# 18281818221/kalle-audio

Measured on AMD Instinct MI355X. Metric: audio-seconds/sec (node) DiT train step, 10s@12.5Hz x1024 latents, higher is better.
Workload: dtype bf16; 1 GPU; DiT train step (fwd+bwd+allreduce+Adam), 24 blocks D=1536 h=24, 10 s @ 12.5 Hz x 1024 latents (T=125+1 prepend), S=130 x 768 cross-attn cond; DiT shape chosen by this build (reference defines none); global_batch=256, per_gpu_batch=256, parallelism=dp1, objective=v, io_channels=1024, global_cond_type=prepend

## Files before the change

### kalle_audio_amd/csrc/gemm2.hip

```cpp
#include <stdio.h>
#include <stdlib.h>
#include <string.h>

#include <algorithm>
#include <functional>
#include <type_traits>
#include <utility>

#include "gemm_common.h"
#include "../../include/kalle_hip.h"

namespace {

constexpr int BK2 = 64;
#define GPTR(p) ((const __attribute__((address_space(1))) void*)(p))

__device__ __attribute__((aligned(64))) const unsigned kalle_zero_block[16] = {0, 0, 0, 0, 0, 0, 0, 0, 0, 0, 0, 0, 0, 0, 0, 0};

template <bool KM, int R, int NW>
struct Loader {
    static constexpr int PER_WAVE = (R / 8) / NW;
    const bf16_t* src[PER_WAVE];
    int64_t kstep;

// ... 56 lines not shown
        if (t == tail_t) issue_tail(region, wave, lane, kvalid);
        else issue(region, wave);
    }
};

template <int OFF>
__device__ __forceinline__ i32x4 lds_b128(unsigned a) {
    i32x4 r;
    asm volatile("ds_read_b128 %0, %1 offset:%2" : "=v"(r) : "v"(a), "n"(OFF));
    return r;
}
__device__ __forceinline__ i32x2 lds_tr(unsigned a) {
    i32x2 r;
    asm volatile("ds_read_b64_tr_b16 %0, %1" : "=v"(r) : "v"(a));
    return r;
}

template <bool KM, int R>
struct Reader {
    unsigned b0[2], b1[2];
    __device__ __forceinline__ void init(int region_off, int rbase, int lane) {
#pragma unroll
        for (int s = 0; s < 2; ++s) {
            if constexpr (!KM) {
                const int row = rbase + (lane & 15);
                const int c = 4 * s + (lane >> 4);
                b0[s] = region_off + row * 128 + ((c ^ ((row >> 1) & 7)) << 4);
                b1[s] = 0;
            } else {
                constexpr int RB = 2 * R;
                const int g = lane >> 4, i = lane & 15;
                const int q = i >> 2, pp = i & 3;
                const int b = 4 * s + g;
                const int odd = b & 1;
                const int pos1 = 8 * b + (odd ? 4 : 0) + q;
                const int pos2 = 8 * b + (odd ? 0 : 4) + q;
                const int cl = (rbase >> 3) + (pp >> 1);
                const int hb = (pp & 1) * 8;
                b0[s] = region_off + pos1 * RB + ((cl ^ (2 * (pos1 & 7))) << 4) + hb;
                b1[s] = region_off + pos2 * RB + ((cl ^ (2 * (pos2 & 7))) << 4) + hb;
            }
        }
    }
    template <int S, int NTILE, int T0 = 0>
    __device__ __forceinline__ void read(unsigned so, i32x4 (&f)[NTILE]) const {
        if constexpr (!KM) {
            const unsigned a = b0[S] + so;
            f[0] = lds_b128<2048 * (T0 + 0)>(a);
            f[1] = lds_b128<2048 * (T0 + 1)>(a);
            f[2] = lds_b128<2048 * (T0 + 2)>(a);
            f[3] = lds_b128<2048 * (T0 + 3)>(a);
            if constexpr (NTILE == 8) {
                f[4] = lds_b128<2048 * (T0 + 4)>(a);
                f[5] = lds_b128<2048 * (T0 + 5)>(a);
                f[6] = lds_b128<2048 * (T0 + 6)>(a);
                f[7] = lds_b128<2048 * (T0 + 7)>(a);
            }
        } else {
            const unsigned a0 = b0[S] + so, a1 = b1[S] + so;
#pragma unroll
            for (int t = 0; t < NTILE; ++t) {
                const i32x2 lo = lds_tr(a0 ^ ((T0 + t) << 5));
                const i32x2 hi = lds_tr(a1 ^ ((T0 + t) << 5));
                f[t] = i32x4{lo[0], lo[1], hi[0], hi[1]};
            }
        }
    }
};

__device__ __forceinline__ void gemm_stamp(const GemmParams& p, int wave, int lane, int idx, int slot = -1) {
    if (p.stamps && (wave == 0 || wave == 7) && lane == 0)
        p.stamps[((int64_t)(slot < 0 ? (int)blockIdx.x : slot) * 2 + (wave ? 1 : 0)) * 8 + idx] = __builtin_amdgcn_s_memrealtime();
}

constexpr int EPI_DEPTH = 1;

struct NoHook { __device__ __forceinline__ void operator()() const {} };

__device__ __forceinline__ int pidx(int r, int c) { return r * 64 + (c ^ ((r & 1) << 2)); }

template <bool C_F32, int TM, int GLU = 0, typename Hook = NoHook>
__device__ __forceinline__ void wave_epilogue(const GemmParams& p, f32x4 (&acc)[TM][4], char* patch_base, int wave, int lane,
                                              int row0, int col0, Hook after_barrier = Hook{}, int stamp_slot = -1) {
    constexpr int DEPTH = EPI_DEPTH < TM ? EPI_DEPTH : TM;
    float* patch = reinterpret_cast<float*>(patch_base) + wave * (16 * 64);
    const int g = lane >> 4, li = lane & 15;
    const bool pre_res = C_F32 && GLU == 0 && !p.atomic && p.residual != nullptr;
    f32x4 rbuf[DEPTH][4];
    auto load_res = [&](int mt, f32x4 (&rv)[4]) {
#pragma unroll
        for (int i = 0; i < 4; ++i) {
            const int gm = row0 + 16 * mt + g + 4 * i, gn = col0 + 4 * li;
            rv[i] = f32x4{0.f, 0.f, 0.f, 0.f};
            if (gm < p.M && gn < p.N) rv[i] = *reinterpret_cast<const f32x4*>(p.residual + gemm_crow(p, gm) * p.ldr + gn);
        }
    };
    i32x4 hbuf[DEPTH][2][2];
    auto load_h = [&](int mt, i32x4 (&hv)[2][2]) {
        const int c8 = (lane & 7) * 8, j0 = col0 + c8;
#pragma unroll
        for (int half = 0; half < 2; ++half) {
            const int gm = row0 + 16 * mt + (lane >> 3) + 8 * half;
            hv[half][0] = i32x4{0, 0, 0, 0};
            hv[half][1] = i32x4{0, 0, 0, 0};
            if (gm < p.M && j0 < p.glu_inner) {
                const bf16_t* hp = static_cast<const bf16_t*>(p.glu_aux) + (int64_t)gm * 2 * p.glu_inner;
                hv[half][0] = *reinterpret_cast<const i32x4*>(hp + j0);
                hv[half][1] = *reinterpret_cast<const i32x4*>(hp + p.glu_inner + j0);
            }
        }
    };
    asm volatile("s_waitcnt lgkmcnt(0)" ::: "memory");
    __builtin_amdgcn_s_barrier();
    after_barrier();
    gemm_stamp(p, wave, lane, 3, stamp_slot);
#pragma unroll
    for (int d = 0; d < DEPTH; ++d) {
        if constexpr (GLU == 2) load_h(d, hbuf[d]);
        if (pre_res) load_res(d, rbuf[d]);
    }
    float sx[8], sg[8];
#pragma unroll
    for (int e = 0; e < 8; ++e) { sx[e] = 0.f; sg[e] = 0.f; }
    f32x4 bias4 = f32x4{0.f, 0.f, 0.f, 0.f}, bias8[2] = {f32x4{0.f, 0.f, 0.f, 0.f}, f32x4{0.f, 0.f, 0.f, 0.f}};
    float bx[8], bg[8];
#pragma unroll
    for (int e = 0; e < 8; ++e) { bx[e] = 0.f; bg[e] = 0.f; }
    if (p.bias) {
        if constexpr (GLU == 1) {
            const int j0 = col0 + (lane & 3) * 8;
            if (j0 < p.glu_inner) {
#pragma unroll
                for (int e = 0; e < 8; ++e) { bx[e] = p.bias[j0 + e]; bg[e] = p.bias[p.glu_inner + j0 + e]; }
            }
        } else if constexpr (GLU == 0) {
            if constexpr (C_F32) {
                if (!p.atomic && col0 + 4 * li < p.N) bias4 = *reinterpret_cast<const f32x4*>(p.bias + col0 + 4 * li);
            } else {
                const int gn = col0 + 8 * (lane & 7);
                if (gn < p.N) {
                    bias8[0] = *reinterpret_cast<const f32x4*>(p.bias + gn);
                    bias8[1] = *reinterpret_cast<const f32x4*>(p.bias + gn + 4);
                }
            }
        }
    }
#pragma unroll
    for (int mt = 0; mt < TM; ++mt) {
        const int slot = mt % DEPTH;
        f32x4 rcur[4];
        i32x4 hcur[2][2];
        if constexpr (GLU == 2) {
#pragma unroll
            for (int half = 0; half < 2; ++half) { hcur[half][0] = hbuf[slot][half][0]; hcur[half][1] = hbuf[slot][half][1]; }
            if (mt + DEPTH < TM) load_h(mt + DEPTH, hbuf[slot]);
        }
        if (pre_res) {
#pragma unroll
            for (int i = 0; i < 4; ++i) rcur[i] = rbuf[slot][i];
            if (mt + DEPTH < TM) load_res(mt + DEPTH, rbuf[slot]);
        }
#pragma unroll
        for (int nt = 0; nt < 4; ++nt)
#pragma unroll
            for (int r = 0; r < 4; ++r) patch[pidx(4 * g + r, 16 * nt + li)] = acc[mt][nt][r];
        asm volatile("s_waitcnt lgkmcnt(0)" ::: "memory");
        const int rbase = row0 + 16 * mt;
        if constexpr (GLU == 1) {
            const int r = lane >> 2, c8 = (lane & 3) * 8;
            const int gm = rbase + r, j0 = col0 + c8;
            if (gm < p.M && j0 < p.glu_inner) {
                float xv[8], gv[8];
#pragma unroll
                for (int e = 0; e < 8; ++e) { xv[e] = patch[pidx(r, c8 + e)]; gv[e] = patch[pidx(r, 32 + c8 + e)]; }
#pragma unroll
                for (int e = 0; e < 8; ++e) { xv[e] += bx[e]; gv[e] += bg[e]; }
                i32x4 hx, hg, av;
#pragma unroll
                for (int e = 0; e < 4; ++e) {
                    hx[e] = (int)pack_bf16x2(xv[2 * e], xv[2 * e + 1]);
                    hg[e] = (int)pack_bf16x2(gv[2 * e], gv[2 * e + 1]);
                    const float x0 = bf16lo((uint32_t)hx[e]), x1 = bf16hi((uint32_t)hx[e]);
                    const float g0 = bf16lo((uint32_t)hg[e]), g1 = bf16hi((uint32_t)hg[e]);
                    av[e] = (int)pack_bf16x2(x0 * siluf_(g0), x1 * siluf_(g1));
                }
                bf16_t* hp = reinterpret_cast<bf16_t*>(p.C) + (int64_t)gm * p.ldc;
                *reinterpret_cast<i32x4*>(hp + j0) = hx;
                *reinterpret_cast<i32x4*>(hp + p.glu_inner + j0) = hg;
                *reinterpret_cast<i32x4*>(static_cast<bf16_t*>(p.glu_aux) + (int64_t)gm * p.glu_inner + j0) = av;
            }
        } else if constexpr (GLU == 2) {
            const int c8 = (lane & 7) * 8, j0 = col0 + c8;
#pragma unroll
            for (int half = 0; half < 2; ++half) {
                const int r = (lane >> 3) + 8 * half;
                const int gm = rbase + r;
                if (gm < p.M && j0 < p.glu_inner) {
                    const i32x4 xv = hcur[half][0], gv = hcur[half][1];
                    i32x4 ox, og;
#pragma unroll
                    for (int e = 0; e < 4; ++e) {
                        const float x[2] = {bf16lo((uint32_t)xv[e]), bf16hi((uint32_t)xv[e])};
                        const float gg[2] = {bf16lo((uint32_t)gv[e]), bf16hi((uint32_t)gv[e])};
                        const float d[2] = {bf16_to_f32(f32_to_bf16(patch[pidx(r, c8 + 2 * e)] * p.alpha)),
                                            bf16_to_f32(f32_to_bf16(patch[pidx(r, c8 + 2 * e + 1)] * p.alpha))};
                        float dx[2], dg[2];
#pragma unroll
                        for (int q = 0; q < 2; ++q) {
                            const float sgm = sigmoidf_(gg[q]);
                            dx[q] = d[q] * gg[q] * sgm;
                            dg[q] = d[q] * x[q] * sgm * (1.f + gg[q] * (1.f - sgm));
                        }
                        ox[e] = (int)pack_bf16x2(dx[0], dx[1]);
                        og[e] = (int)pack_bf16x2(dg[0], dg[1]);
                        sx[2 * e] += bf16lo((uint32_t)ox[e]); sx[2 * e + 1] += bf16hi((uint32_t)ox[e]);
                        sg[2 * e] += bf16lo((uint32_t)og[e]); sg[2 * e + 1] += bf16hi((uint32_t)og[e]);
                    }
                    bf16_t* dp = reinterpret_cast<bf16_t*>(p.C) + (int64_t)gm * p.ldc;
                    *reinterpret_cast<i32x4*>(dp + j0) = ox;
                    *reinterpret_cast<i32x4*>(dp + p.glu_inner + j0) = og;
                }
            }
        } else if (p.atomic) {
            const int gn = col0 + lane;
#pragma unroll 4
            for (int r = 0; r < 16; ++r) {
                const int gm = rbase + r;
                if (gm < p.M && gn < p.N)
                    atomicAdd(reinterpret_cast<float*>(p.C) + (int64_t)gm * p.ldc + gn, patch[pidx(r, lane)] * p.alpha);
            }
        } else if constexpr (C_F32) {
#pragma unroll
            for (int i = 0; i < 4; ++i) {
                const int r = g + 4 * i;
                const int gm = rbase + r, gn = col0 + 4 * li;
                if (gm >= p.M || gn >= p.N) continue;
                const f32x4 pv = *reinterpret_cast<const f32x4*>(patch + pidx(r, 4 * li));
                float v[4] = {pv[0], pv[1], pv[2], pv[3]};
                const int64_t crow = gemm_crow(p, gm);
                gemm_epilogue4(p, gm, gn, crow, v, false, &bias4);
                if (pre_res) {
#pragma unroll
                    for (int j = 0; j < 4; ++j) v[j] += rcur[i][j];
                }
                float* cp = reinterpret_cast<float*>(p.C) + crow * p.ldc + gn;
                if (p.accumulate) {
                    const f32x4 c0 = *reinterpret_cast<const f32x4*>(cp);
#pragma unroll
                    for (int j = 0; j < 4; ++j) v[j] += c0[j];
                }
                *reinterpret_cast<f32x4*>(cp) = f32x4{v[0], v[1], v[2], v[3]};
            }
        } else {
#pragma unroll
            for (int half = 0; half < 2; ++half) {
                const int r = (lane >> 3) + 8 * half;
                const int gm = rbase + r, gn = col0 + 8 * (lane & 7);
                if (gm >= p.M || gn >= p.N) continue;
                const f32x4 p0 = *reinterpret_cast<const f32x4*>(patch + pidx(r, 8 * (lane & 7)));
                const f32x4 p1 = *reinterpret_cast<const f32x4*>(patch + pidx(r, 8 * (lane & 7) + 4));
                float v0[4] = {p0[0], p0[1], p0[2], p0[3]}, v1[4] = {p1[0], p1[1], p1[2], p1[3]};
                const int64_t crow = gemm_crow(p, gm);
                gemm_epilogue4(p, gm, gn, crow, v0, true, &bias8[0]);
                gemm_epilogue4(p, gm, gn + 4, crow, v1, true, &bias8[1]);
                i32x4 o;
                o[0] = (int)pack_bf16x2(v0[0], v0[1]);
                o[1] = (int)pack_bf16x2(v0[2], v0[3]);
                o[2] = (int)pack_bf16x2(v1[0], v1[1]);
                o[3] = (int)pack_bf16x2(v1[2], v1[3]);
                *reinterpret_cast<i32x4*>(reinterpret_cast<bf16_t*>(p.C) + crow * p.ldc + gn) = o;
            }
        }
        asm volatile("s_waitcnt lgkmcnt(0)" ::: "memory");
    }
    if constexpr (GLU == 2) {
        if (p.glu_dbias) {
#pragma unroll
            for (int e = 0; e < 8; ++e) {
#pragma unroll
                for (int o = 8; o < 64; o <<= 1) { sx[e] += __shfl_xor(sx[e], o, 64); sg[e] += __shfl_xor(sg[e], o, 64); }
            }
            const int j0 = col0 + (lane & 7) * 8;
            if (lane < 8 && j0 < p.glu_inner) {
#pragma unroll
                for (int e = 0; e < 8; ++e) {
                    atomicAdd(p.glu_dbias + j0 + e, sx[e]);
                    atomicAdd(p.glu_dbias + p.glu_inner + j0 + e, sg[e]);
                }
            }
        }
    }
    if (p.stamps) {
        gemm_stamp(p, wave, lane, 4, stamp_slot);
        asm volatile("s_waitcnt vmcnt(0)" ::: "memory");
        gemm_stamp(p, wave, lane, 5, stamp_slot);
    }
}

#define MFMA16(FA, FB)                                                                                         \
    _Pragma("unroll") for (int mt = 0; mt < 4; ++mt) _Pragma("unroll") for (int nt = 0; nt < 4; ++nt)          \
        acc[mt][nt] = __builtin_amdgcn_mfma_f32_16x16x32_bf16(__builtin_bit_cast(bf16x8, FA[mt]),              \
                                                              __builtin_bit_cast(bf16x8, FB[nt]), acc[mt][nt], 0, 0, 0)

template <bool A_KM, bool B_KM, bool C_F32, int WM, int WN, int TM, int GLU = 0, int NS = 3>
__global__ __launch_bounds__(WM * WN * 64, 2) void gemm2_kernel(GemmParams p) {
    static_assert(TM == 4, "wave tile is 64 x 64");
    constexpr int TN = 4;
    constexpr int NW = WM * WN;
    constexpr int BM = WM * TM * 16, BN = WN * TN * 16;
    constexpr int A_BYTES = BM * 128, B_BYTES = BN * 128, STAGE = A_BYTES + B_BYTES;
    extern __shared__ __attribute__((aligned(16))) char smem[];
    const unsigned lds0 = (unsigned)(size_t)LDS_PTR(char, smem);

    const int tid = threadIdx.x, lane = tid & 63;
    const int wave = __builtin_amdgcn_readfirstlane(tid >> 6);
    const int wm = wave / WN, wn = wave % WN;

    int tm, tn;
    gemm_tile_coords(blockIdx.x, gridDim.x, p.tiles_m, p.tiles_n, p.group_m, tm, tn);
    const int m0 = tm * BM, n0 = tn * BN;

    const int nk_all = (p.K + BK2 - 1) / BK2;
    const int kt0 = blockIdx.y * p.ktiles_per_split;
    const int nk = min(p.ktiles_per_split, nk_all - kt0);
    const int kvalid = p.K % BK2;
    const int tail_t = kvalid ? nk_all - 1 - kt0 : -1;

    f32x4 acc[TM][TN];
#pragma unroll
    for (int i = 0; i < TM; ++i)
#pragma unroll
        for (int j = 0; j < TN; ++j) acc[i][j] = f32x4{0.f, 0.f, 0.f, 0.f};

    Loader<A_KM, BM, NW> la;
    Loader<B_KM, BN, NW> lb;
    la.init(p.A, p.lda, p.M, m0, kt0 * BK2, wave, lane);
    lb.init(p.B, p.ldb, p.N, n0, kt0 * BK2, wave, lane, GLU == 1 ? p.glu_inner : 0, tn);
    const int arow = wm * TM * 16, bcol = wn * TN * 16;
    Reader<A_KM, BM> ra;
    Reader<B_KM, BN> rb;
    ra.init(lds0, arow, lane);
    rb.init(lds0 + A_BYTES, bcol, lane);

    {
    constexpr int PT = Loader<A_KM, BM, NW>::PER_WAVE + Loader<B_KM, BN, NW>::PER_WAVE;
    static_assert((NS - 2) * PT <= 63, "vmcnt is a 6-bit counter");
    {
        const int pre = nk < NS ? nk : NS;
#pragma unroll
        for (int t = 0; t < NS; ++t) {
            if (t < pre) {
                la.issue_at(smem + t * STAGE, wave, lane, t, tail_t, kvalid);
                lb.issue_at(smem + t * STAGE + A_BYTES, wave, lane, t, tail_t, kvalid);
            }
        }
        constexpr int PRE_KEEP = (NS - 1) * PT <= 63 ? NS - 1 : NS - 2;
        const int keep = pre - 1 < PRE_KEEP ? pre - 1 : PRE_KEEP;
        auto wait_keep = [&](auto self, auto c) {
            constexpr int C = decltype(c)::value;
            if (keep == C) asm volatile("s_waitcnt vmcnt(%0)" ::"n"(C * PT) : "memory");
            if constexpr (C > 0) self(self, std::integral_constant<int, C - 1>{});
        };
        wait_keep(wait_keep, std::integral_constant<int, PRE_KEEP>{});
    }
    __builtin_amdgcn_s_barrier();
    __builtin_amdgcn_sched_barrier(0);

    i32x4 fa0[4], fb0[4], fa1[4], fb1[4];
    ra.template read<0, 4>(0, fa0);
    rb.template read<0, 4>(0, fb0);

    unsigned so_cur = 0, so_nxt = STAGE;
    int kt = 0;

    auto iteration = [&](auto issue_c, auto next_c, auto keep_c) {
        constexpr bool ISSUE = decltype(issue_c)::value, NEXT = decltype(next_c)::value;
        constexpr int KEEP = decltype(keep_c)::value;
        asm volatile("s_waitcnt lgkmcnt(0)" ::: "memory");
        __builtin_amdgcn_sched_barrier(0);
// ... 210 lines not shown
template <bool A_KM, bool B_KM, bool C_F32, int WM, int WN, int TM, int GLU = 0, int NS = 3>
int launch2(const GemmParams& p, hipStream_t st) {
    constexpr int BM = WM * TM * 16, BN = WN * 64;
    constexpr int lds = NS * (BM + BN) * 128;
    static_assert(lds <= 160 * 1024, "LDS per workgroup");
    static std::atomic<uint64_t> lds_ok{0};
    kalle_allow_lds(reinterpret_cast<const void*>(gemm2_kernel<A_KM, B_KM, C_F32, WM, WN, TM, GLU, NS>), lds, lds_ok);
    dim3 grid(p.tiles_m * p.tiles_n, p.splits), block(WM * WN * 64);
    KALLE_LAUNCH((gemm2_kernel<A_KM, B_KM, C_F32, WM, WN, TM, GLU, NS>), grid, block, lds, st, p);
    return kalle_check_launch();
}



constexpr int GEMM3_LDS = 2 * (256 + 256) * 128 + 8 * 16 * 64 * 4;

static int kalle_cu_count() {
    static std::atomic<int> cached[64];
    int dev = 0;
    (void)hipGetDevice(&dev);
    int v = cached[dev & 63].load(std::memory_order_relaxed);
    if (v > 0) return v;
    hipDeviceProp_t prop;
    v = hipGetDeviceProperties(&prop, dev) == hipSuccess && prop.multiProcessorCount > 0 ? prop.multiProcessorCount : 256;
    v &= ~7;
    if (v < 8) v = 8;
    cached[dev & 63].store(v, std::memory_order_relaxed);
    return v;
}

#define MFMA32(FA, FB)                                                                                         \
    _Pragma("unroll") for (int mt = 0; mt < 8; ++mt) _Pragma("unroll") for (int nt = 0; nt < 4; ++nt)          \
        acc[mt][nt] = __builtin_amdgcn_mfma_f32_16x16x32_bf16(__builtin_bit_cast(bf16x8, FA[mt]),              \
                                                              __builtin_bit_cast(bf16x8, FB[nt]), acc[mt][nt], 0, 0, 0)

constexpr int SCHED_SETS = 256;
constexpr int SCHED_LINE = 32;
__device__ int kalle_gemm_sched[SCHED_SETS][9 * SCHED_LINE];

__device__ __forceinline__ int sched_issue(int* sched, int xcd) { return atomicAdd(sched + xcd * SCHED_LINE, 1); }
__device__ __forceinline__ int sched_resolve(int xcd, int raw, int first_round, int ntiles) {
    const int id = xcd + 8 * (first_round + raw);
    return id < ntiles ? id : ntiles;
}
__device__ __forceinline__ void sched_leave(int* sched, int nwg) {
    if (atomicAdd(sched + 8 * SCHED_LINE, 1) == nwg - 1) {
#pragma unroll
        for (int i = 0; i < 9; ++i) atomicExch(sched + i * SCHED_LINE, 0);
    }
}

template <bool A_KM, bool B_KM, bool C_F32, int GLU, bool XCD_RASTER, bool PERSIST>
__device__ __forceinline__ void gemm3_tiles(const GemmParams& p, int tile0, int tstride, int tile_end, int ntiles_raster, int kt0,
                                            int nk) {
    const int kvalid = p.K % BK2;
    const int tail_t = kvalid ? (p.K + BK2 - 1) / BK2 - 1 - kt0 : -1;
    constexpr int WN = 4, TM = 8, NW = 8;
    constexpr int BM = 256, BN = 256;
    constexpr int A_BYTES = BM * 128, B_BYTES = BN * 128, STAGE = A_BYTES + B_BYTES;
    extern __shared__ __attribute__((aligned(16))) char smem[];
    const unsigned lds0 = (unsigned)(size_t)LDS_PTR(char, smem);

    const int tid = threadIdx.x, lane = tid & 63;
    const int wave = __builtin_amdgcn_readfirstlane(tid >> 6);
    const int wm = wave / WN, wn = wave % WN;
    const int arow = wm * 128, bcol = wn * 64;
    Loader<A_KM, BM, NW> la;
    Loader<B_KM, BN, NW> lb;
    Reader<A_KM, BM> ra;
    Reader<B_KM, BN> rb;
    ra.init(lds0, arow, lane);
    rb.init(lds0 + A_BYTES, bcol, lane);
    const bool late = wave >= NW / 2;
    if (late) __builtin_amdgcn_s_setprio(1);

    auto coords = [&](int tile, int& tm, int& tn) {
        if constexpr (XCD_RASTER) gemm_tile_coords(tile, ntiles_raster, p.tiles_m, p.tiles_n, p.group_m, tm, tn);
        else gemm_tile_coords_plain(tile, p.tiles_m, p.tiles_n, p.group_m, tm, tn);
    };
    auto init_loaders = [&](int tm, int tn, int kt_first) {
        la.init(p.A, p.lda, p.M, tm * BM, (kt0 + kt_first) * BK2, wave, lane);
        lb.init(p.B, p.ldb, p.N, tn * BN, (kt0 + kt_first) * BK2, wave, lane, GLU == 1 ? p.glu_inner : 0, tn);
    };
    bool prefetched = false;
    unsigned s0 = 0;

    int* const sched = PERSIST && p.sched_set > 0 ? &kalle_gemm_sched[p.sched_set - 1][0] : nullptr;
    int next_tile = tile_end;
    int drawn = 0;
    if constexpr (PERSIST) {
        if (sched && tid == 0) drawn = sched_issue(sched, blockIdx.x & 7);
    }
    volatile int* const mailbox = reinterpret_cast<volatile int*>(smem + 2 * STAGE);
    for (int tile = tile0; tile < tile_end; tile = next_tile) {
        int tm, tn;
        coords(tile, tm, tn);
        const int m0 = tm * BM, n0 = tn * BN;
        next_tile = PERSIST ? tile + tstride : tile_end;
        bool has_next = PERSIST && next_tile < tile_end;
        gemm_stamp(p, wave, lane, 0, tile);
        f32x4 acc[TM][4];
#pragma unroll
        for (int i = 0; i < TM; ++i)
#pragma unroll
            for (int j = 0; j < 4; ++j) acc[i][j] = f32x4{0.f, 0.f, 0.f, 0.f};

        if (!prefetched) {
            init_loaders(tm, tn, 0);
            la.issue_at(smem, wave, lane, 0, tail_t, kvalid);
            lb.issue_at(smem + A_BYTES, wave, lane, 0, tail_t, kvalid);
            s0 = 0;
            if (nk > 1) {
                la.issue_at(smem + STAGE, wave, lane, 1, tail_t, kvalid);
                lb.issue_at(smem + STAGE + A_BYTES, wave, lane, 1, tail_t, kvalid);
                asm volatile("s_waitcnt vmcnt(8)" ::: "memory");
            } else {
                asm volatile("s_waitcnt vmcnt(0)" ::: "memory");
            }
        } else if constexpr (PERSIST) {
            init_loaders(tm, tn, nk > 1 ? 2 : 1);
            asm volatile("s_waitcnt vmcnt(0)" ::: "memory");
        }
        if constexpr (PERSIST) {
            if (sched && tid == 0) {
                *mailbox = sched_resolve(blockIdx.x & 7, drawn, tstride >> 3, tile_end);
                asm volatile("s_waitcnt lgkmcnt(0)" ::: "memory");
            }
        }
        __builtin_amdgcn_s_barrier();
        __builtin_amdgcn_sched_barrier(0);
        if constexpr (PERSIST) {
            if (sched) {
                next_tile = __builtin_amdgcn_readfirstlane(*mailbox);
                has_next = next_tile < tile_end;
            }
        }
        gemm_stamp(p, wave, lane, 1, tile);

        i32x4 fa[8], fb[4];
        unsigned so_cur = s0;
        int kt = 0;
        ra.template read<0, 8>(so_cur, fa);
        rb.template read<0, 4>(so_cur, fb);

        auto iteration = [&](auto issue_c, auto next_c) {
            constexpr bool ISSUE = decltype(issue_c)::value, NEXT = decltype(next_c)::value;
            asm volatile("s_waitcnt lgkmcnt(0)" ::: "memory");
            __builtin_amdgcn_sched_barrier(0);
            MFMA32(fa, fb);
            __builtin_amdgcn_sched_barrier(0);
            ra.template read<1, 8>(so_cur, fa);
            rb.template read<1, 4>(so_cur, fb);
            asm volatile("s_waitcnt lgkmcnt(0)" ::: "memory");
            __builtin_amdgcn_sched_barrier(0);
            if (!late) {
                MFMA32(fa, fb);
                __builtin_amdgcn_sched_barrier(0);
            }
            asm volatile("s_waitcnt vmcnt(0)" ::: "memory");
            __builtin_amdgcn_s_barrier();
            __builtin_amdgcn_sched_barrier(0);
            if (late) {
                MFMA32(fa, fb);
                __builtin_amdgcn_sched_barrier(0);
            }
            if constexpr (ISSUE) {
                la.issue_at(smem + so_cur, wave, lane, kt + 2, tail_t, kvalid);
                lb.issue_at(smem + so_cur + A_BYTES, wave, lane, kt + 2, tail_t, kvalid);
            }
            so_cur ^= STAGE;
            if constexpr (NEXT) {
                ra.template read<0, 8>(so_cur, fa);
                rb.template read<0, 4>(so_cur, fb);
            }
            __builtin_amdgcn_sched_barrier(0);
        };
        auto last_iteration = [&]() {
            asm volatile("s_waitcnt lgkmcnt(0)" ::: "memory");
            __builtin_amdgcn_sched_barrier(0);
            MFMA32(fa, fb);
            __builtin_amdgcn_sched_barrier(0);
            ra.template read<1, 8>(so_cur, fa);
            rb.template read<1, 4>(so_cur, fb);
            asm volatile("s_waitcnt lgkmcnt(0)" ::: "memory");
            __builtin_amdgcn_sched_barrier(0);
            MFMA32(fa, fb);
            __builtin_amdgcn_sched_barrier(0);
        };
        using T_ = std::true_type;
        using F_ = std::false_type;
#pragma unroll 1
        for (; kt + 2 < nk; ++kt) iteration(T_{}, T_{});
        if (kt + 1 < nk) { iteration(F_{}, T_{}); ++kt; }
        if constexpr (!PERSIST || GLU == 2) iteration(F_{}, F_{});
        else last_iteration();
        gemm_stamp(p, wave, lane, 2, tile);

        const unsigned s_last = so_cur;
        auto hook = [&]() {
            if constexpr (!PERSIST) return;
            if (has_next) {
                int ntm, ntn;
                coords(next_tile, ntm, ntn);
                init_loaders(ntm, ntn, 0);
                la.issue_at(smem + (s_last ^ STAGE), wave, lane, 0, tail_t, kvalid);
                lb.issue_at(smem + (s_last ^ STAGE) + A_BYTES, wave, lane, 0, tail_t, kvalid);
                if (nk > 1) {
                    la.issue_at(smem + s_last, wave, lane, 1, tail_t, kvalid);
                    lb.issue_at(smem + s_last + A_BYTES, wave, lane, 1, tail_t, kvalid);
                }
                if (sched && tid == 0) drawn = sched_issue(sched, blockIdx.x & 7);
            }
        };
        wave_epilogue<C_F32, TM, GLU>(p, acc, smem + 2 * STAGE, wave, lane, m0 + arow, GLU == 1 ? tn * 128 + wn * 32 : n0 + bcol,
                                      hook, tile);
        prefetched = has_next;
        s0 = s_last ^ STAGE;
        if constexpr (!PERSIST) break;
    }
}

template <bool A_KM, bool B_KM, bool C_F32, int GLU = 0>
__global__ __launch_bounds__(512, 2) void gemm3_kernel(GemmParams p) {
    const int nk_all = (p.K + BK2 - 1) / BK2;
    const int ntiles = p.tiles_m * p.tiles_n;
    if constexpr (A_KM) {
        if (p.mix_na >= 0) {
            const int na = p.mix_na, sa = p.mix_sa;
            int bid = blockIdx.x, tile, slice, per;
            if (bid < na * sa) { tile = bid % na; slice = bid / na; per = (nk_all + sa - 1) / sa; }
            else { bid -= na * sa; const int nb = ntiles - na; tile = na + bid % nb; slice = bid / nb; per = (nk_all + sa) / (sa + 1); }
            const int kt0 = slice * per, nk = min(per, nk_all - kt0);
            if (nk <= 0) return;
            gemm3_tiles<A_KM, B_KM, C_F32, GLU, true, false>(p, tile, 0, tile + 1, ntiles, kt0, nk);
        } else {
            const int kt0 = blockIdx.y * p.ktiles_per_split;
            gemm3_tiles<A_KM, B_KM, C_F32, GLU, true, false>(p, blockIdx.x, 0, blockIdx.x + 1, ntiles, kt0,
                                                             min(p.ktiles_per_split, nk_all - kt0));
        }
    } else {
        gemm3_tiles<A_KM, B_KM, C_F32, GLU, true, true>(p, blockIdx.x, gridDim.x, ntiles, ntiles, 0, nk_all);
        if (p.sched_set > 0 && threadIdx.x == 0) sched_leave(&kalle_gemm_sched[p.sched_set - 1][0], gridDim.x);
    }
}

struct GroupProblem {
    const bf16_t* A;
    const bf16_t* B;
    float* C;
    int64_t lda, ldb, ldc;
    int M, N, K;
    int tiles_m, tiles_n, group_m;
    int unsplit, splits;
    int r1_start, r2_start;
};
struct GroupParams {
    int nprob, r2_base;
    int overwrite;
    GroupProblem pr[KALLE_MAX_GROUP];
};

__global__ __launch_bounds__(256) void gemm3_group_zero_kernel(GroupParams gp) {
    int pi = 0, base = 0;
    const int bid = blockIdx.x >> 2, band = blockIdx.x & 3;
    for (;;) {
        const int nb = gp.pr[pi].tiles_m * gp.pr[pi].tiles_n - gp.pr[pi].unsplit;
        if (bid < base + nb || pi + 1 >= gp.nprob) break;
        base += nb;
        ++pi;
    }
    const GroupProblem& q = gp.pr[pi];
    int tm, tn;
    gemm_tile_coords_plain(q.unsplit + bid - base, q.tiles_m, q.tiles_n, q.group_m, tm, tn);
    const int r0 = tm * 256 + band * 64, c0 = tn * 256;
    for (int i = threadIdx.x; i < 64 * 64; i += 256) {
        const int r = r0 + i / 64, c = c0 + (i & 63) * 4;
        if (r < q.M && c < q.N) *reinterpret_cast<f32x4*>(q.C + (int64_t)r * q.ldc + c) = f32x4{0.f, 0.f, 0.f, 0.f};
    }
}

__global__ __launch_bounds__(512, 2) void gemm3_wgrad_group_kernel(GroupParams gp) {
    const bool whole = (int)blockIdx.x < gp.r2_base;
    const int bid = whole ? xcd_contiguous(blockIdx.x, gp.r2_base)
                          : gp.r2_base + xcd_contiguous(blockIdx.x - gp.r2_base, gridDim.x - gp.r2_base);
    int pi = 0, tile, slice = 0;
    if (whole) {
        while (pi + 1 < gp.nprob && bid >= gp.pr[pi + 1].r1_start) ++pi;
        tile = bid - gp.pr[pi].r1_start;
    } else {
        while (pi + 1 < gp.nprob && bid >= gp.pr[pi + 1].r2_start) ++pi;
        const int local = bid - gp.pr[pi].r2_start, nb = gp.pr[pi].tiles_m * gp.pr[pi].tiles_n - gp.pr[pi].unsplit;
        tile = gp.pr[pi].unsplit + local % nb;
        slice = local / nb;
    }
    const GroupProblem& q = gp.pr[pi];
    GemmParams p{};
    p.A = q.A; p.B = q.B; p.C = q.C;
    p.lda = q.lda; p.ldb = q.ldb; p.ldc = q.ldc;
// ... 574 lines not shown
```

### kalle_audio_amd/csrc/gemm_common.h

```cpp
#pragma once
#include "common.h"

struct GemmParams {
    const bf16_t* A;
    const bf16_t* B;
    void* C;
    int64_t lda, ldb, ldc;
    int M, N, K;
    const float* bias;
    const float* gate;
    int64_t ldg;
    int rows_per_batch;
    const float* residual;
    int64_t ldr;
    int accumulate;
    int tiles_n;
    float alpha;
    int c_rpb, c_brows, c_roff;
    const uint8_t* row_mask;
    int tiles_m, splits, ktiles_per_split, atomic, group_m, tile_n;
    int mix_na, mix_sa;
    int glu_mode, glu_inner;
    void* glu_aux;
    float* glu_dbias;
    int64_t slab_stride;
    unsigned long long* stamps;
    int sched_set;
};

__device__ __forceinline__ void gemm_tile_coords(int bid, int nwg, int tiles_m, int tiles_n, int gm, int& tm, int& tn) {
    const int qd = nwg >> 3, rm = nwg & 7, xcd = bid & 7;
    const int wg = (xcd < rm ? xcd * (qd + 1) : rm * (qd + 1) + (xcd - rm) * qd) + (bid >> 3);
    const int per_group = gm * tiles_n;
    const int group = wg / per_group;
    const int first_m = group * gm;
    const int gsz = min(gm, tiles_m - first_m);
    const int in = wg - group * per_group;
    tm = first_m + in % gsz;
    tn = in / gsz;
}

__device__ __forceinline__ int xcd_contiguous(int bid, int nwg) {
    const int qd = nwg >> 3, rm = nwg & 7, xcd = bid & 7;
    return (xcd < rm ? xcd * (qd + 1) : rm * (qd + 1) + (xcd - rm) * qd) + (bid >> 3);
}

__device__ __forceinline__ void gemm_tile_coords_plain(int wg, int tiles_m, int tiles_n, int gm, int& tm, int& tn) {
    const int per_group = gm * tiles_n;
    const int group = wg / per_group;
    const int first_m = group * gm;
    const int gsz = min(gm, tiles_m - first_m);
    const int in = wg - group * per_group;
    tm = first_m + in % gsz;
    tn = in / gsz;
}

__device__ __forceinline__ int64_t gemm_crow(const GemmParams& p, int gm) {
    return p.c_rpb > 0 ? (int64_t)(gm / p.c_rpb) * p.c_brows + p.c_roff + gm % p.c_rpb : gm;
}

__device__ __forceinline__ void gemm_epilogue4(const GemmParams& p, int gm, int gn, int64_t crow, float (&v)[4],
                                               bool with_residual = true, const f32x4* bias_pre = nullptr) {
#pragma unroll
    for (int j = 0; j < 4; ++j) v[j] *= p.alpha;
    if (p.bias) {
        const f32x4 b = bias_pre ? *bias_pre : *reinterpret_cast<const f32x4*>(p.bias + gn);
#pragma unroll
        for (int j = 0; j < 4; ++j) v[j] += b[j];
    }
    if (p.gate) {
        const f32x4 g = *reinterpret_cast<const f32x4*>(p.gate + (int64_t)(gm / p.rows_per_batch) * p.ldg + gn);
#pragma unroll
        for (int j = 0; j < 4; ++j) v[j] *= sigmoidf_(1.f - g[j]);
    }
    if (p.row_mask && !p.row_mask[gm]) {
#pragma unroll
        for (int j = 0; j < 4; ++j) v[j] = 0.f;
    }
    if (with_residual && p.residual) {
        const f32x4 r = *reinterpret_cast<const f32x4*>(p.residual + crow * p.ldr + gn);
#pragma unroll
        for (int j = 0; j < 4; ++j) v[j] += r[j];
    }
}

struct GemmLayout { bool a_km = false, b_km = false, f32 = false; };

struct GemmPlan {
    int family = 0;
    GemmLayout lay;
    int wm = 0, wn = 0;
    int tile_n = 0, tiles_m = 0, tiles_n = 0, group_m = 0;
    int splits = 0, ktiles_per_split = 0;
    int mix_na = -1, mix_sa = 0;
    int atomic = 0;
    bool clear_c = false;
    bool slabs = false;
    int word = 0;
};

static inline int gemm_plan_word(const GemmPlan& g) {
    if (g.family == 5) return 5 | (g.wm << 8) | (g.wn << 12) | (g.splits << 16);
    if (g.family == 4) return 4 | (1 << 8);
    return g.family | (g.splits << 8) | (g.mix_na >= 0 ? 1 << 24 : 0);
}

int launch_gemm_v1(const GemmParams& p, bool a_km, bool b_km, bool f32, hipStream_t st);
```

Measured before the change: 11690 audio-seconds/sec.

## Stream epilogue residual/SwiGLU operands through an LDS ring via async global-to-LDS loads

Adds a ring-buffered epilogue for persistent fp32-residual GEMMs and the fused SwiGLU backward. It prefetches residual or saved h tiles into spare LDS stage space with global_load_lds, two row-tiles ahead, and hoists gate, bias and row-mask loads out of the per-row loop. The next tile's second K-stage load is deferred until the ring slots are released, and the scheduler mailbox is moved into LDS. The aim is to hide epilogue global-load latency behind the accumulator writeback, at the cost of more complex vmcnt accounting and a later start for the next tile's prefetch.

Result: no change. 11770 audio-seconds/sec (median of 6 runs) (+0.7%).

```diff
diff --git a/kalle_audio_amd/csrc/gemm2.hip b/kalle_audio_amd/csrc/gemm2.hip
--- a/kalle_audio_amd/csrc/gemm2.hip
+++ b/kalle_audio_amd/csrc/gemm2.hip
@@ -162,6 +162,7 @@
 template <bool C_F32, int TM, int GLU = 0, typename Hook = NoHook>
 __device__ __forceinline__ void wave_epilogue(const GemmParams& p, f32x4 (&acc)[TM][4], char* patch_base, int wave, int lane,
                                               int row0, int col0, Hook after_barrier = Hook{}, int stamp_slot = -1) {
+    static_assert(GLU != 2, "the fused SwiGLU backward runs on wave_epilogue_ring");
     constexpr int DEPTH = EPI_DEPTH < TM ? EPI_DEPTH : TM;
     float* patch = reinterpret_cast<float*>(patch_base) + wave * (16 * 64);
     const int g = lane >> 4, li = lane & 15;
@@ -175,33 +176,14 @@
             if (gm < p.M && gn < p.N) rv[i] = *reinterpret_cast<const f32x4*>(p.residual + gemm_crow(p, gm) * p.ldr + gn);
         }
     };
-    i32x4 hbuf[DEPTH][2][2];
-    auto load_h = [&](int mt, i32x4 (&hv)[2][2]) {
-        const int c8 = (lane & 7) * 8, j0 = col0 + c8;
-#pragma unroll
-        for (int half = 0; half < 2; ++half) {
-            const int gm = row0 + 16 * mt + (lane >> 3) + 8 * half;
-            hv[half][0] = i32x4{0, 0, 0, 0};
-            hv[half][1] = i32x4{0, 0, 0, 0};
-            if (gm < p.M && j0 < p.glu_inner) {
-                const bf16_t* hp = static_cast<const bf16_t*>(p.glu_aux) + (int64_t)gm * 2 * p.glu_inner;
-                hv[half][0] = *reinterpret_cast<const i32x4*>(hp + j0);
-                hv[half][1] = *reinterpret_cast<const i32x4*>(hp + p.glu_inner + j0);
-            }
-        }
-    };
     asm volatile("s_waitcnt lgkmcnt(0)" ::: "memory");
     __builtin_amdgcn_s_barrier();
     after_barrier();
     gemm_stamp(p, wave, lane, 3, stamp_slot);
 #pragma unroll
     for (int d = 0; d < DEPTH; ++d) {
-        if constexpr (GLU == 2) load_h(d, hbuf[d]);
         if (pre_res) load_res(d, rbuf[d]);
     }
-    float sx[8], sg[8];
-#pragma unroll
-    for (int e = 0; e < 8; ++e) { sx[e] = 0.f; sg[e] = 0.f; }
     f32x4 bias4 = f32x4{0.f, 0.f, 0.f, 0.f}, bias8[2] = {f32x4{0.f, 0.f, 0.f, 0.f}, f32x4{0.f, 0.f, 0.f, 0.f}};
     float bx[8], bg[8];
 #pragma unroll
@@ -229,12 +211,6 @@
     for (int mt = 0; mt < TM; ++mt) {
         const int slot = mt % DEPTH;
         f32x4 rcur[4];
-        i32x4 hcur[2][2];
-        if constexpr (GLU == 2) {
-#pragma unroll
-            for (int half = 0; half < 2; ++half) { hcur[half][0] = hbuf[slot][half][0]; hcur[half][1] = hbuf[slot][half][1]; }
-            if (mt + DEPTH < TM) load_h(mt + DEPTH, hbuf[slot]);
-        }
         if (pre_res) {
 #pragma unroll
             for (int i = 0; i < 4; ++i) rcur[i] = rbuf[slot][i];
@@ -268,38 +244,6 @@
                 *reinterpret_cast<i32x4*>(hp + j0) = hx;
                 *reinterpret_cast<i32x4*>(hp + p.glu_inner + j0) = hg;
                 *reinterpret_cast<i32x4*>(static_cast<bf16_t*>(p.glu_aux) + (int64_t)gm * p.glu_inner + j0) = av;
-            }
-        } else if constexpr (GLU == 2) {
-            const int c8 = (lane & 7) * 8, j0 = col0 + c8;
-#pragma unroll
-            for (int half = 0; half < 2; ++half) {
-                const int r = (lane >> 3) + 8 * half;
-                const int gm = rbase + r;
-                if (gm < p.M && j0 < p.glu_inner) {
-                    const i32x4 xv = hcur[half][0], gv = hcur[half][1];
-                    i32x4 ox, og;
-#pragma unroll
-                    for (int e = 0; e < 4; ++e) {
-                        const float x[2] = {bf16lo((uint32_t)xv[e]), bf16hi((uint32_t)xv[e])};
-                        const float gg[2] = {bf16lo((uint32_t)gv[e]), bf16hi((uint32_t)gv[e])};
-                        const float d[2] = {bf16_to_f32(f32_to_bf16(patch[pidx(r, c8 + 2 * e)] * p.alpha)),
-                                            bf16_to_f32(f32_to_bf16(patch[pidx(r, c8 + 2 * e + 1)] * p.alpha))};
-                        float dx[2], dg[2];
-#pragma unroll
-                        for (int q = 0; q < 2; ++q) {
-                            const float sgm = sigmoidf_(gg[q]);
-                            dx[q] = d[q] * gg[q] * sgm;
-                            dg[q] = d[q] * x[q] * sgm * (1.f + gg[q] * (1.f - sgm));
-                        }
-                        ox[e] = (int)pack_bf16x2(dx[0], dx[1]);
-                        og[e] = (int)pack_bf16x2(dg[0], dg[1]);
-                        sx[2 * e] += bf16lo((uint32_t)ox[e]); sx[2 * e + 1] += bf16hi((uint32_t)ox[e]);
-                        sg[2 * e] += bf16lo((uint32_t)og[e]); sg[2 * e + 1] += bf16hi((uint32_t)og[e]);
-                    }
-                    bf16_t* dp = reinterpret_cast<bf16_t*>(p.C) + (int64_t)gm * p.ldc;
-                    *reinterpret_cast<i32x4*>(dp + j0) = ox;
-                    *reinterpret_cast<i32x4*>(dp + p.glu_inner + j0) = og;
-                }
             }
         } else if (p.atomic) {
             const int gn = col0 + lane;
@@ -353,6 +297,181 @@
         }
         asm volatile("s_waitcnt lgkmcnt(0)" ::: "memory");
     }
+    if (p.stamps) {
+        gemm_stamp(p, wave, lane, 4, stamp_slot);
+        asm volatile("s_waitcnt vmcnt(0)" ::: "memory");
+        gemm_stamp(p, wave, lane, 5, stamp_slot);
+    }
+}
+
+__device__ __forceinline__ unsigned lds_addr(const void* q) { return (unsigned)(size_t)LDS_PTR(char, q); }
+__device__ __forceinline__ f32x4 lds_read16(unsigned a) {
+    f32x4 r;
+    asm volatile("ds_read_b128 %0, %1" : "=v"(r) : "v"(a) : "memory");
+    return r;
+}
+__device__ __forceinline__ void lds_write4(unsigned a, float v) { asm volatile("ds_write_b32 %0, %1" ::"v"(a), "v"(v) : "memory"); }
+__device__ __forceinline__ void lds_wait(f32x4 (&a)[4], f32x4 (&b)[4]) {
+    asm volatile("s_waitcnt lgkmcnt(0)"
+                 : "+v"(a[0]), "+v"(a[1]), "+v"(a[2]), "+v"(a[3]), "+v"(b[0]), "+v"(b[1]), "+v"(b[2]), "+v"(b[3])::"memory");
+}
+
+template <int TM, int GLU, typename Hook, typename Tail>
+__device__ __forceinline__ void wave_epilogue_ring(const GemmParams& p, f32x4 (&acc)[TM][4], char* patch_base, char* ring0, char* ring1,
+                                                   int wave, int lane, int row0, int col0, Hook after_barrier, Tail ring_free,
+                                                   int stamp_slot) {
+    static_assert(GLU == 0 || GLU == 2, "fp32 residual or fused SwiGLU backward");
+    static_assert(TM >= 2, "two ring slots");
+    asm volatile("" : "+v"(lane));
+    const int g = lane >> 4, li = lane & 15;
+    const unsigned pa = lds_addr(patch_base) + wave * (16 * 64 * 4);
+    char* const ring[2] = {ring0, ring1};
+    const unsigned ra[2] = {lds_addr(ring0) + 16 * lane, lds_addr(ring1) + 16 * lane};
+    const int ncols = GLU == 2 ? p.glu_inner : p.N;
+    const bool cols_full = col0 + 64 <= ncols;
+    const unsigned pw_even = pa + 4 * pidx(4 * g, li), pw_odd = pa + 4 * pidx(4 * g + 1, li);
+
+    auto fetch = [&](int mt) {
+#pragma unroll
+        for (int i = 0; i < 4; ++i) {
+            const void* sp = kalle_zero_block;
+            if constexpr (GLU == 2) {
+                const int gm = row0 + 16 * mt + (lane >> 3) + 8 * (i >> 1), j0 = col0 + (lane & 7) * 8;
+                if (gm < p.M && j0 < p.glu_inner)
+                    sp = static_cast<const bf16_t*>(p.glu_aux) + (int64_t)gm * 2 * p.glu_inner + (i & 1) * p.glu_inner + j0;
+            } else {
+                const int gm = row0 + 16 * mt + g + 4 * i, gn = col0 + 4 * li;
+                if (gm < p.M && gn < p.N) sp = p.residual + gemm_crow(p, gm) * p.ldr + gn;
+            }
+            __builtin_amdgcn_global_load_lds(GPTR(sp), LDS_PTR(void, ring[mt & 1] + 1024 * i), 16, 0, 0);
+        }
+    };
+
+    const bool alpha1 = p.alpha == 1.f;
+    float sx[8], sg[8];
+#pragma unroll
+    for (int e = 0; e < 8; ++e) { sx[e] = 0.f; sg[e] = 0.f; }
+
+    asm volatile("s_waitcnt lgkmcnt(0)" ::: "memory");
+    __builtin_amdgcn_s_barrier();
+    after_barrier();
+    gemm_stamp(p, wave, lane, 3, stamp_slot);
+    fetch(0);
+    fetch(1);
+    f32x4 bias4 = f32x4{0.f, 0.f, 0.f, 0.f}, gq[3] = {bias4, bias4, bias4};
+    int b0 = 0;
+    unsigned long long mask_even = ~0ull, mask_odd = ~0ull;
+    if constexpr (GLU == 0) {
+        const int gn = col0 + 4 * li;
+        if (p.bias && gn < p.N) bias4 = *reinterpret_cast<const f32x4*>(p.bias + gn);
+        if (p.gate) {
+            const int blast = (p.M - 1) / p.rows_per_batch;
+            b0 = min(row0 / p.rows_per_batch, blast);
+            if (gn < p.N) {
+#pragma unroll
+                for (int k = 0; k < 3; ++k) gq[k] = *reinterpret_cast<const f32x4*>(p.gate + (int64_t)min(b0 + k, blast) * p.ldg + gn);
+            }
+        }
+        if (p.row_mask) {
+            const int r = row0 + 2 * lane;
+            const int me = r < p.M ? (int)p.row_mask[r] : 0, mo = r + 1 < p.M ? (int)p.row_mask[r + 1] : 0;
+            mask_even = __ballot(me != 0);
+            mask_odd = __ballot(mo != 0);
+        }
+    }
+    if constexpr (GLU == 0) __builtin_amdgcn_s_waitcnt(0x0F70);
+#pragma unroll
+    for (int mt = 0; mt < TM; ++mt) {
+        const int rbase = row0 + 16 * mt;
+#pragma unroll
+        for (int nt = 0; nt < 4; ++nt)
+#pragma unroll
+            for (int r = 0; r < 4; ++r) lds_write4(((r & 1) ? pw_odd - 256 : pw_even) + 256 * r + 64 * nt, acc[mt][nt][r]);
+        if (mt + 1 < TM) {
+            if (mt > 0 && cols_full && rbase <= p.M) asm volatile("s_waitcnt vmcnt(8)" ::: "memory");
+            else asm volatile("s_waitcnt vmcnt(4)" ::: "memory");
+        } else {
+            if (cols_full && rbase <= p.M) asm volatile("s_waitcnt vmcnt(4)" ::: "memory");
+            else asm volatile("s_waitcnt vmcnt(0)" ::: "memory");
+        }
+        f32x4 opv[4], pv[4];
+#pragma unroll
+        for (int i = 0; i < 4; ++i) opv[i] = lds_read16(ra[mt & 1] + 1024 * i);
+        if constexpr (GLU == 2) {
+            const int c8 = (lane & 7) * 8;
+#pragma unroll
+            for (int half = 0; half < 2; ++half) {
+                const int r = (lane >> 3) + 8 * half;
+                pv[2 * half] = lds_read16(pa + 4 * pidx(r, c8));
+                pv[2 * half + 1] = lds_read16(pa + 4 * pidx(r, c8 + 4));
+            }
+        } else {
+#pragma unroll
+            for (int i = 0; i < 4; ++i) pv[i] = lds_read16(pa + 4 * pidx(g + 4 * i, 4 * li));
+        }
+        lds_wait(opv, pv);
+        if (mt + 2 < TM) fetch(mt + 2);
+        if constexpr (GLU == 2) {
+            const int c8 = (lane & 7) * 8, j0 = col0 + c8;
+            if (!alpha1) {
+#pragma unroll
+                for (int q = 0; q < 4; ++q)
+#pragma unroll
+                    for (int e = 0; e < 4; ++e) pv[q][e] *= p.alpha;
+            }
+#pragma unroll
+            for (int half = 0; half < 2; ++half) {
+                const int r = (lane >> 3) + 8 * half;
+                const int gm = rbase + r;
+                if (gm < p.M && j0 < p.glu_inner) {
+                    const i32x4 xv = __builtin_bit_cast(i32x4, opv[2 * half]), gv = __builtin_bit_cast(i32x4, opv[2 * half + 1]);
+                    i32x4 ox, og;
+#pragma unroll
+                    for (int e = 0; e < 4; ++e) {
+                        const float x[2] = {bf16lo((uint32_t)xv[e]), bf16hi((uint32_t)xv[e])};
+                        const float gg[2] = {bf16lo((uint32_t)gv[e]), bf16hi((uint32_t)gv[e])};
+                        const float d[2] = {bf16_to_f32(f32_to_bf16(pv[2 * half + (e >> 1)][2 * (e & 1)])),
+                                            bf16_to_f32(f32_to_bf16(pv[2 * half + (e >> 1)][2 * (e & 1) + 1]))};
+                        float dx[2], dg[2];
+#pragma unroll
+                        for (int q = 0; q < 2; ++q) {
+#pragma clang fp reassociate(off)
+                            const float sgm = sigmoidf_(gg[q]);
+                            const float ds = sgm * d[q];
+                            dx[q] = ds * gg[q];
+                            dg[q] = (__builtin_fmaf(1.f - sgm, gg[q], 1.f) * x[q]) * ds;
+                        }
+                        ox[e] = (int)pack_bf16x2(dx[0], dx[1]);
+                        og[e] = (int)pack_bf16x2(dg[0], dg[1]);
+                        sx[2 * e] += bf16lo((uint32_t)ox[e]); sx[2 * e + 1] += bf16hi((uint32_t)ox[e]);
+                        sg[2 * e] += bf16lo((uint32_t)og[e]); sg[2 * e + 1] += bf16hi((uint32_t)og[e]);
+                    }
+                    bf16_t* dp = reinterpret_cast<bf16_t*>(p.C) + (int64_t)gm * p.ldc;
+                    *reinterpret_cast<i32x4*>(dp + j0) = ox;
+                    *reinterpret_cast<i32x4*>(dp + p.glu_inner + j0) = og;
+                }
+            }
+        } else {
+#pragma unroll
+            for (int i = 0; i < 4; ++i) {
+                const int rel = 16 * mt + g + 4 * i;
+                const int gm = row0 + rel, gn = col0 + 4 * li;
+                if (gm >= p.M || gn >= p.N) continue;
+                float v[4] = {pv[i][0], pv[i][1], pv[i][2], pv[i][3]};
+                const int64_t crow = gemm_crow(p, gm);
+                f32x4 gate4 = gq[0];
+                if (p.gate) {
+                    const int k = gm / p.rows_per_batch - b0;
+                    gate4 = k == 0 ? gq[0] : k == 1 ? gq[1] : gq[2];
+                }
+                const int keep = (int)(((rel & 1) ? mask_odd : mask_even) >> (rel >> 1)) & 1;
+                gemm_epilogue4(p, gm, gn, crow, v, false, &bias4, &gate4, keep);
+#pragma unroll
+                for (int j = 0; j < 4; ++j) v[j] += opv[i][j];
+                *reinterpret_cast<f32x4*>(reinterpret_cast<float*>(p.C) + crow * p.ldc + gn) = f32x4{v[0], v[1], v[2], v[3]};
+            }
+        }
+    }
     if constexpr (GLU == 2) {
         if (p.glu_dbias) {
 #pragma unroll
@@ -375,6 +494,7 @@
         asm volatile("s_waitcnt vmcnt(0)" ::: "memory");
         gemm_stamp(p, wave, lane, 5, stamp_slot);
     }
+    ring_free();
 }
 
 #define MFMA16(FA, FB)                                                                                         \
@@ -751,6 +871,9 @@
         la.init(p.A, p.lda, p.M, tm * BM, (kt0 + kt_first) * BK2, wave, lane);
         lb.init(p.B, p.ldb, p.N, tn * BN, (kt0 + kt_first) * BK2, wave, lane, GLU == 1 ? p.glu_inner : 0, tn);
     };
+    constexpr bool HEAVY = PERSIST && ((!A_KM && !B_KM && C_F32 && GLU == 0) || GLU == 2);
+    static_assert(GLU != 2 || PERSIST, "the fused SwiGLU backward runs whole-K tiles");
+    bool k1_late = false;
     bool prefetched = false;
     unsigned s0 = 0;
 
@@ -788,19 +911,38 @@
             }
         } else if constexpr (PERSIST) {
             init_loaders(tm, tn, nk > 1 ? 2 : 1);
-            asm volatile("s_waitcnt vmcnt(0)" ::: "memory");
-        }
-        if constexpr (PERSIST) {
+            if constexpr (HEAVY) {
+                if (k1_late) asm volatile("s_waitcnt vmcnt(8)" ::: "memory");
+                else asm volatile("s_waitcnt vmcnt(0)" ::: "memory");
+            } else {
+                asm volatile("s_waitcnt vmcnt(0)" ::: "memory");
+            }
+        }
+        if constexpr (PERSIST && !HEAVY) {
             if (sched && tid == 0) {
                 *mailbox = sched_resolve(blockIdx.x & 7, drawn, tstride >> 3, tile_end);
                 asm volatile("s_waitcnt lgkmcnt(0)" ::: "memory");
             }
         }
+        if constexpr (HEAVY) {
+            if (sched && tid == 0) {
+                lds_write4(lds_addr(smem + 2 * STAGE), __builtin_bit_cast(float, sched_resolve(blockIdx.x & 7, drawn, tstride >> 3, tile_end)));
+                asm volatile("s_waitcnt lgkmcnt(0)" ::: "memory");
+            }
+        }
         __builtin_amdgcn_s_barrier();
         __builtin_amdgcn_sched_barrier(0);
-        if constexpr (PERSIST) {
+        if constexpr (PERSIST && !HEAVY) {
             if (sched) {
                 next_tile = __builtin_amdgcn_readfirstlane(*mailbox);
+                has_next = next_tile < tile_end;
+            }
+        }
+        if constexpr (HEAVY) {
+            if (sched) {
+                int v;
+                asm volatile("ds_read_b32 %0, %1\n\ts_waitcnt lgkmcnt(0)" : "=v"(v) : "v"(lds_addr(smem + 2 * STAGE)) : "memory");
+                next_tile = __builtin_amdgcn_readfirstlane(v);
                 has_next = next_tile < tile_end;
             }
         }
@@ -866,23 +1008,58 @@
         gemm_stamp(p, wave, lane, 2, tile);
 
         const unsigned s_last = so_cur;
-        auto hook = [&]() {
-            if constexpr (!PERSIST) return;
-            if (has_next) {
-                int ntm, ntn;
+        if constexpr (!HEAVY) {
+            auto hook = [&]() {
+                if constexpr (!PERSIST) return;
+                if (has_next) {
+                    int ntm, ntn;
+                    coords(next_tile, ntm, ntn);
+                    init_loaders(ntm, ntn, 0);
+                    la.issue_at(smem + (s_last ^ STAGE), wave, lane, 0, tail_t, kvalid);
+                    lb.issue_at(smem + (s_last ^ STAGE) + A_BYTES, wave, lane, 0, tail_t, kvalid);
+                    if (nk > 1) {
+                        la.issue_at(smem + s_last, wave, lane, 1, tail_t, kvalid);
+                        lb.issue_at(smem + s_last + A_BYTES, wave, lane, 1, tail_t, kvalid);
+                    }
+                    if (sched && tid == 0) drawn = sched_issue(sched, blockIdx.x & 7);
+                }
+            };
+            wave_epilogue<C_F32, TM, GLU>(p, acc, smem + 2 * STAGE, wave, lane, m0 + arow, GLU == 1 ? tn * 128 + wn * 32 : n0 + bcol,
+                                          hook, tile);
+        } else {
+            const bool ring = GLU == 2 || (!p.atomic && !p.accumulate && p.residual != nullptr && (!p.gate || p.rows_per_batch >= 64));
+            auto request = [&](int kt, unsigned so) {
+                int ntm, ntn, ln = lane;
                 coords(next_tile, ntm, ntn);
-                init_loaders(ntm, ntn, 0);
-                la.issue_at(smem + (s_last ^ STAGE), wave, lane, 0, tail_t, kvalid);
-                lb.issue_at(smem + (s_last ^ STAGE) + A_BYTES, wave, lane, 0, tail_t, kvalid);
-                if (nk > 1) {
-                    la.issue_at(smem + s_last, wave, lane, 1, tail_t, kvalid);
-                    lb.issue_at(smem + s_last + A_BYTES, wave, lane, 1, tail_t, kvalid);
+                asm volatile("" : "+v"(ln));
+                la.init(p.A, p.lda, p.M, ntm * BM, (kt0 + kt) * BK2, wave, ln);
+                lb.init(p.B, p.ldb, p.N, ntn * BN, (kt0 + kt) * BK2, wave, ln);
+                la.issue_at(smem + so, wave, lane, kt, tail_t, kvalid);
+                lb.issue_at(smem + so + A_BYTES, wave, lane, kt, tail_t, kvalid);
+            };
+            auto hook = [&]() {
+                if (has_next) {
+                    request(0, s_last ^ STAGE);
+                    if (nk > 1 && !ring) request(1, s_last);
+                    if (sched && tid == 0) drawn = sched_issue(sched, blockIdx.x & 7);
                 }
-                if (sched && tid == 0) drawn = sched_issue(sched, blockIdx.x & 7);
-            }
-        };
-        wave_epilogue<C_F32, TM, GLU>(p, acc, smem + 2 * STAGE, wave, lane, m0 + arow, GLU == 1 ? tn * 128 + wn * 32 : n0 + bcol,
-                                      hook, tile);
+            };
+            auto ring_free = [&]() {
+                if (has_next && nk > 1) request(1, s_last);
+            };
+            k1_late = ring && has_next && nk > 1;
+            char* const ring0 = smem + s_last + wave * 4096;
+            if constexpr (GLU == 2) {
+                wave_epilogue_ring<TM, 2>(p, acc, smem + 2 * STAGE, ring0, ring0 + A_BYTES, wave, lane, m0 + arow, n0 + bcol, hook,
+                                          ring_free, tile);
+            } else {
+                if (ring)
+                    wave_epilogue_ring<TM, 0>(p, acc, smem + 2 * STAGE, ring0, ring0 + A_BYTES, wave, lane, m0 + arow, n0 + bcol, hook,
+                                              ring_free, tile);
+                else
+                    wave_epilogue<C_F32, TM, GLU>(p, acc, smem + 2 * STAGE, wave, lane, m0 + arow, n0 + bcol, hook, tile);
+            }
+        }
         prefetched = has_next;
         s0 = s_last ^ STAGE;
         if constexpr (!PERSIST) break;
diff --git a/kalle_audio_amd/csrc/gemm_common.h b/kalle_audio_amd/csrc/gemm_common.h
--- a/kalle_audio_amd/csrc/gemm_common.h
+++ b/kalle_audio_amd/csrc/gemm_common.h
@@ -60,7 +60,8 @@
 }
 
 __device__ __forceinline__ void gemm_epilogue4(const GemmParams& p, int gm, int gn, int64_t crow, float (&v)[4],
-                                               bool with_residual = true, const f32x4* bias_pre = nullptr) {
+                                               bool with_residual = true, const f32x4* bias_pre = nullptr,
+                                               const f32x4* gate_pre = nullptr, int mask_pre = -1) {
 #pragma unroll
     for (int j = 0; j < 4; ++j) v[j] *= p.alpha;
     if (p.bias) {
@@ -69,11 +70,11 @@
         for (int j = 0; j < 4; ++j) v[j] += b[j];
     }
     if (p.gate) {
-        const f32x4 g = *reinterpret_cast<const f32x4*>(p.gate + (int64_t)(gm / p.rows_per_batch) * p.ldg + gn);
+        const f32x4 g = gate_pre ? *gate_pre : *reinterpret_cast<const f32x4*>(p.gate + (int64_t)(gm / p.rows_per_batch) * p.ldg + gn);
 #pragma unroll
         for (int j = 0; j < 4; ++j) v[j] *= sigmoidf_(1.f - g[j]);
     }
-    if (p.row_mask && !p.row_mask[gm]) {
+    if (p.row_mask && !(mask_pre >= 0 ? mask_pre : (int)p.row_mask[gm])) {
 #pragma unroll
         for (int j = 0; j < 4; ++j) v[j] = 0.f;
     }
```
